# pouryashirazian/FemBrain

Hardware: AMD Instinct MI355X
Metric: FEM steps/sec (assemble+PCG) at 1M tets (higher is better)
Workload: dtype f64 arithmetic / f32 stored matrix

## Files before the change

### fembrain_amd/csrc/pcg_pipe.hip.h

```cpp
#pragma once
#include "fem_kernels.h"
#include "pcg_pipe_stream.hip.h"
#include "pcg_pipe_onchip.hip.h"
#include "pcg_pipe_mirror.h"
#include "pcg_pipe_regs.hip.h"

namespace fb {

constexpr int kPipeMaxWaves = 12;
constexpr int kPipeMaxBlocks = 256;
constexpr int kPipeSyncDoubles = 2 * 16 + 2 * kPipeMaxBlocks + 8;
constexpr int kPipeMaxProducers = 64;
constexpr int pipe_slot_bytes(bool c16) { return c16 ? 9 * 256 + 128 : 10 * 256; }
constexpr int pipe_lds_slots(bool c16) { return c16 ? 65 : 62; }
static_assert(sizeof(double) * kPipeSyncDoubles + (size_t)pipe_lds_slots(false) * pipe_slot_bytes(false) <= 160 * 1024, "LDS budget of k_pcg_pipe");
static_assert(sizeof(double) * kPipeSyncDoubles + (size_t)pipe_lds_slots(true) * pipe_slot_bytes(true) <= 160 * 1024, "LDS budget of k_pcg_pipe<c16>");
static_assert(mir_slot_bytes(true) == pipe_slot_bytes(true) && mir_slot_bytes(false) == pipe_slot_bytes(false) && mir_lds_slots(true) == pipe_lds_slots(true) &&
              mir_lds_slots(false) == pipe_lds_slots(false) && kMirWaves == kPipeMaxWaves, "the LDS window's planner sees the kernel's LDS");
static_assert(pipe_lds_slots(true) * pipe_slot_bytes(true) / 4 < 65536 && pipe_lds_slots(false) * pipe_slot_bytes(false) / 4 < 65536, "16-bit LDS word addresses of the mirror layers");

struct PipeArgs {
  unsigned long long* post;
  unsigned int* flags;
  unsigned int* error;
// ... 177 lines not shown
    if (lane == 0) { mw[w].d = d; mw[w].m = m; mw[w].width = width; }
  }
  __syncthreads();
  if (threadIdx.x == 0) ok = count > 0 && mir_wg_layout(mw, count, klt, c16, 0, false) ? 1 : 0;
  __syncthreads();
  for (int pass = 0; pass < 2; pass++) {
    if (ok && w < count) {
      int e = 0;
      for (int k = 0; k < mw[w].m; k++) e += __popcll(__ballot(mir_lane_addr(slice_off, colidx, first, mw, w, k, lane, lo, hi, c16) < 0));
      if (lane == 0) cnt[w] = e;
    }
    __syncthreads();
    if (threadIdx.x == 0 && ok) {
      int E = 0;
      for (int v = 0; v < count; v++) E += cnt[v];
      if (pass == 0) ok = E <= kMirPoolMax && mir_wg_layout(mw, count, klt, c16, E, true) ? 1 : 0;
      else ok = mir_wg_gains(mw, count, klt, c16) ? 1 : 0;
    }
    __syncthreads();
  }
  if (threadIdx.x == 0) {
    if (!ok) mir_wg_plain(mw, count, klt, c16);
    int E = 0, layers = 0, fewest = 1 << 30, held = 0;
    for (int v = 0; v < count; v++) {
      const int e = ok ? cnt[v] : 0;
      cnt[v] = E;
      E += e; layers += mw[v].m; fewest = min(fewest, mw[v].p); held += mir_reg_slots(mw[v], regs);
    }
    if (held > 0) atomicAdd(&stats[3], held);
    wg_out[b] = make_int2(mir_pool_at(mw, count, c16) / 4, E);
    atomicAdd(&stats[0], layers); atomicAdd(&stats[1], E);
    if (count > 0) atomicMin(&stats[2], fewest);
  }
  __syncthreads();
  if (w < count) {
    const int sl = first + w, pool_at = mir_pool_at(mw, count, c16) / 4;
    int e = cnt[w];
    for (int k = 0; k < mw[w].m; k++) {
      int addr = mir_lane_addr(slice_off, colidx, first, mw, w, k, lane, lo, hi, c16);
      const unsigned long long miss = __ballot(addr < 0);
      if (addr < 0) {
        const int idx = e + __popcll(miss & ((1ULL << lane) - 1ULL));
        pool_src[(size_t)b * kMirPoolMax + idx] = (slice_off[sl] + mw[w].a + k) * 9 * 64 + lane;
        addr = pool_at + (idx >> 6) * 9 * 64 + (idx & 63);
      }
      e += __popcll(miss);
      addr_out[((size_t)sl * kMirMax + k) * 64 + lane] = (unsigned short)addr;
    }
  }
  if (w < kMirWaves && lane == 0)
    wave_out[(size_t)b * kMirWaves + w] = w < count ? make_int4(mw[w].a | mw[w].m << 8 | mw[w].p << 16, mw[w].at, mw[w].tab, mir_reg_slots(mw[w], regs)) : make_int4(0, 0, 0, 0);
}

template <bool SERVE_PRIO = false>
__device__ __forceinline__ void pipe_collect_posts(const PipeArgs& pa, unsigned int sums, int nb, int lane, int stride, int l0, long long t0, long long t_limit, bool& failed,
                                                   double& t0s, double& t1s) {
  const unsigned long long* post = pa.post + (size_t)(sums & 1u) * nb * 4;
  for (int b = l0; b - lane < nb && !failed; b += stride) {
    const bool mine = b < nb;
    uint4 q4[2] = {make_uint4(0, 0, 0, 0), make_uint4(0, 0, 0, 0)};
    for (;;) {
      bool ok = true;
      if (mine) {
        asm volatile("global_load_dwordx4 %0, %2, off sc1\n\tglobal_load_dwordx4 %1, %2, off offset:16 sc1\n\ts_waitcnt vmcnt(0)"
                     : "=&v"(q4[0]), "=&v"(q4[1]) : "v"(post + (size_t)b * 4) : "memory");
        ok = q4[0].y == sums && q4[0].w == sums && q4[1].y == sums && q4[1].w == sums;
      }
      if (__ballot(!ok) == 0ULL) break;
      if constexpr (SERVE_PRIO) pipe_setprio<0>();
      if (ld_sc1_u32(pa.error) != 0u || wall_clock64() - t0 > t_limit) { failed = true; break; }
      __builtin_amdgcn_s_sleep(1);
    }
    if constexpr (SERVE_PRIO) pipe_setprio<1>();
    if (mine && !failed) {
      t0s += __longlong_as_double((long long)(((unsigned long long)q4[0].x << 32) | (unsigned long long)q4[0].z));
      t1s += __longlong_as_double((long long)(((unsigned long long)q4[1].x << 32) | (unsigned long long)q4[1].z));
    }
  }
}

__global__ __launch_bounds__(256) void k_gather_lines(int n_slices, int step, const int* __restrict__ slice_off, const int* __restrict__ colidx,
                                                      unsigned long long* __restrict__ out) {
  const int lane = threadIdx.x & 63;
  const int wave = (int)((blockIdx.x * blockDim.x + threadIdx.x) >> 6), n_waves = (int)((gridDim.x * blockDim.x) >> 6);
  unsigned long long planes = 0, records = 0, slots = 0;
  for (int s = wave * step; s < n_slices; s += n_waves * step) {
    for (int slot = slice_off[s]; slot < slice_off[s + 1]; slot++) {
      const unsigned int col = (unsigned int)colidx[(size_t)slot * 64 + lane];
      const unsigned int kp = col >> 4, k0 = (col * 24u) >> 7, k1 = (col * 24u + 23u) >> 7;
      bool first_p = true, first_0 = true, first_1 = k1 != k0;
      for (int l = 0; l < 64; l++) {
        const unsigned int op = __builtin_amdgcn_readlane(kp, l), o0 = __builtin_amdgcn_readlane(k0, l), o1 = __builtin_amdgcn_readlane(k1, l);
        if (l < lane) {
          first_p = first_p && op != kp;
          first_0 = first_0 && o0 != k0 && o1 != k0;
          first_1 = first_1 && o0 != k1 && o1 != k1;
        }
      }
      planes += __popcll(__ballot(first_p));
      records += __popcll(__ballot(first_0)) + __popcll(__ballot(first_1));
      slots++;
    }
  }
  if (lane == 0 && slots) { atomicAdd(out, planes); atomicAdd(out + 1, records); atomicAdd(out + 2, slots); }
}

}
#include "pcg_shard_box.hip.h"
namespace fb {

}
#define FB_PIPE_KERNEL k_pcg_pipe
#define FB_PIPE_KERNEL_ATTR
#define FB_PIPE_KERNEL_HOLDS false
#include "pcg_pipe_kernel.h"
#undef FB_PIPE_KERNEL
#undef FB_PIPE_KERNEL_ATTR
#undef FB_PIPE_KERNEL_HOLDS
#define FB_PIPE_KERNEL k_pcg_pipe_regs
#define FB_PIPE_KERNEL_ATTR __attribute__((amdgpu_num_vgpr(FB_PIPE_REGS_VGPR_PAIRS)))
#define FB_PIPE_KERNEL_HOLDS true
#include "pcg_pipe_kernel.h"
#undef FB_PIPE_KERNEL
// ... 3 lines not shown
```

### fembrain_amd/csrc/pcg_pipe2.hip.h

```cpp
#pragma once
#include "pcg_pipe.hip.h"

namespace fb {

constexpr int kPipe2LdsWordsPerRow = 24;
constexpr int kPipe2SliceBytes = kPipe2LdsWordsPerRow * 64 * 4;
constexpr int kPipe2Klt = 4;
__host__ __device__ constexpr int pipe2_lds_slots(int count, bool c16) {
  return (160 * 1024 - (int)sizeof(double) * kPipeSyncDoubles - (count + 1) * kPipe2SliceBytes) / pipe_slot_bytes(c16) > 0
             ? (160 * 1024 - (int)sizeof(double) * kPipeSyncDoubles - (count + 1) * kPipe2SliceBytes) / pipe_slot_bytes(c16) : 0;
}

template <bool C16, bool SHARD, bool XYZ = false>
__global__ __launch_bounds__(64 * kPipeMaxWaves) void k_pcg_pipe2(SellView sv, const float* __restrict__ vals, const float* __restrict__ dlo,
                                                                  const double* __restrict__ invdiag, const double* __restrict__ bvec,
                                                                  double* __restrict__ xg, double* __restrict__ rg, double* __restrict__ wg,
                                                                  double* __restrict__ zg, double* __restrict__ sg, double* __restrict__ pg,
                                                                  CGState* __restrict__ st, PipeArgs pa, ShardArgs sa) {
  static_assert(!SHARD || !C16, "a shard's columns are 32-bit local ids");
  static_assert(!SHARD || !XYZ, "a shard publishes planes");
  extern __shared__ double lds[];
  double* wsum = lds;
  double* gath = lds + 32;
  double* bc = gath + 2 * kPipeMaxBlocks;
// ... 41 lines not shown
#pragma unroll
      for (int j = 0; j < 9; j++) lv[(k * kValWords + j) * 64] = __float_as_uint(vk[j * 64]);
      if constexpr (C16) lc[k * 64] = sv.coldelta[((size_t)so[h] + k) * 64 + lane];
      else lv[(k * 10 + 9) * 64] = (unsigned int)sv.colidx[((size_t)so[h] + k) * 64 + lane];
    }
  }
  double iv[2][3] = {{0, 0, 0}, {0, 0, 0}};
#pragma unroll
  for (int h = 0; h < 2; h++) {
    float m6[6] = {0, 0, 0, 0, 0, 0};
    if (rvalid[h]) {
      const float* l = dlo + (size_t)(row[h] >> 6) * 9 * 64 + lane;
      m6[0] = l[0 * 64]; m6[1] = l[1 * 64]; m6[2] = l[2 * 64]; m6[3] = l[4 * 64]; m6[4] = l[5 * 64]; m6[5] = l[8 * 64];
#pragma unroll
      for (int a = 0; a < 3; a++) iv[h][a] = invdiag[3 * (size_t)row[h] + a];
    }
#pragma unroll
    for (int k = 0; k < 6; k++) *lds_f(h, k) = m6[k];
#pragma unroll
    for (int k = 0; k < 9; k++) *lds_d(h, k) = 0.0;
  }
  const int n_prod = pa.prod_count[blockIdx.x];
  int my_prod = -1;
  if (wv == 0 && n_prod >= 0 && lane < n_prod) my_prod = pa.producers[(size_t)blockIdx.x * kPipeMaxProducers + lane];

  unsigned int send_mask = 0u;
  ShardBoxLayout BL = {};
  if constexpr (SHARD) { send_mask = sa.wg_send_mask[blockIdx.x]; BL = shard_box_layout(sa.halo_cap); }
  unsigned int pub = pa.seqs[0], sums = pa.seqs[1];
  const long long t_limit = pa.timeout_ticks;
  bool failed = false;

  const size_t xs = XYZ ? 1 : pa.n_pad, cs = XYZ ? 3 : 1;
  auto publish = [&](const double vin[2][3]) {
    pub++;
    double* pl = pa.planes + (size_t)(pub & 1u) * 3 * pa.n_pad;
#pragma unroll
    for (int h = 0; h < 2; h++)
      if (rvalid[h]) {
        if constexpr (XYZ) {
          st_sc1_xyz(pl + 3 * (size_t)row[h], vin[h][0], vin[h][1], vin[h][2]);
        } else {
#pragma unroll
          for (int a = 0; a < 3; a++) st_sc1_f64(pl + a * xs + cs * (size_t)row[h], vin[h][a]);
        }
        if constexpr (SHARD) shard_send_row(sa, BL, pub, send_beg[h], send_end[h], vin[h]);
      }
  };
  auto product = [&](const double vin[2][3], double y[2][3], bool post_sums, bool late_acquire) {
    double* pl = pa.planes + (size_t)(pub & 1u) * 3 * pa.n_pad;
    asm volatile("s_waitcnt vmcnt(0)" ::: "memory");
    __syncthreads();
    if (post_sums) sums++;
    if (wv != 0 && live[0] && pa.prefetch_slots > 0 && width[0] > KL[0]) {
      int so_k = so[0] + KL[0];
      asm volatile("" : "+s"(so_k));
      pipe_prefetch_values(min(pa.prefetch_slots, width[0] - KL[0]), ((unsigned int)so_k * 9u * 64u + (unsigned int)lane) * (unsigned int)sizeof(float), vals);
    }
    if constexpr (SHARD) {
      if (spare) shard_service_product(sa, BL, pa, pub, pl, nb, lane, send_mask, t_limit, bc, failed);
    }
    if (wv == 0) {
      if (lane == 0) st_sc1_u32(pa.flags + blockIdx.x, pub);
      if (post_sums && lane < 2) {
        double t = 0.0;
        for (int w = 0; w < n_waves; w++) t += wsum[lane * 16 + w];
        const unsigned long long bits = (unsigned long long)__double_as_longlong(t), tag = (unsigned long long)sums << 32;
        unsigned long long* post = pa.post + ((size_t)(sums & 1u) * nb + blockIdx.x) * 4 + 2 * lane;
        st_sc1_u64(post, (bits >> 32) | tag);
        st_sc1_u64(post + 1, (bits & 0xffffffffULL) | tag);
      }
      if (!late_acquire) __builtin_amdgcn_fence(__ATOMIC_ACQUIRE, "agent");
      const long long t0 = wall_clock64();
      if (n_prod >= 0) {
        for (;;) {
          bool ok = true;
          if (my_prod >= 0) ok = (int)(ld_sc1_u32(pa.flags + my_prod) - pub) >= 0;
          if (__ballot(!ok) == 0ULL) break;
          if (ld_sc1_u32(pa.error) != 0u || wall_clock64() - t0 > t_limit) { failed = true; break; }
          __builtin_amdgcn_s_sleep(1);
        }
      } else if constexpr (SHARD) {
        shard_poll_all(sa, pa, pub, nb, lane, t0, t_limit, failed);
      } else {
        for (int b = 4 * lane; b - 4 * lane < nb && !failed; b += 256) {
          for (;;) {
            bool ok = true;
            if (b < nb) {
              const uint4 f = ld_sc1_u128(pa.flags + b);
              ok = (int)(f.x - pub) >= 0 && (b + 1 >= nb || (int)(f.y - pub) >= 0) && (b + 2 >= nb || (int)(f.z - pub) >= 0) && (b + 3 >= nb || (int)(f.w - pub) >= 0);
            }
            if (__ballot(!ok) == 0ULL) break;
            if (ld_sc1_u32(pa.error) != 0u || wall_clock64() - t0 > t_limit) { failed = true; break; }
            __builtin_amdgcn_s_sleep(1);
          }
        }
      }
      if (failed && lane == 0) st_sc1_u32(pa.error, 1u);
      if (late_acquire) __builtin_amdgcn_fence(__ATOMIC_ACQUIRE, "agent");
      asm volatile("s_waitcnt vmcnt(0)" ::: "memory");
      if (lane == 0) bc[3] = (failed || ld_sc1_u32(pa.error) != 0u) ? 1.0 : 0.0;
    }
    __syncthreads();
    if (uniform_flag(bc[3] != 0.0 || (SHARD && bc[4] != 0.0))) { failed = true; return; }
#pragma unroll
    for (int h = 0; h < 2; h++) {
      double y0 = 0, y1 = 0, y2 = 0;
      if (rvalid[h]) {
        const double l00 = (double)*lds_f(h, 0), l01 = (double)*lds_f(h, 1), l02 = (double)*lds_f(h, 2), l11 = (double)*lds_f(h, 3), l12 = (double)*lds_f(h, 4),
                     l22 = (double)*lds_f(h, 5);
        y0 = l00 * vin[h][0] + l01 * vin[h][1] + l02 * vin[h][2];
        y1 = l01 * vin[h][0] + l11 * vin[h][1] + l12 * vin[h][2];
        y2 = l02 * vin[h][0] + l12 * vin[h][1] + l22 * vin[h][2];
      }
      if (live[h]) {
        const unsigned int* lv = (const unsigned int*)lres[h] + lane;
        const short* lc = (const short*)(lres[h] + (size_t)klt[h] * 9 * 256) + lane;
#pragma unroll
        for (int k = 0; k < kPipe2Klt; k++) if (k < KL[h]) {
          const unsigned int* lk = lv + (size_t)k * kValWords * 64;
          unsigned int col;
          if constexpr (C16) col = (unsigned int)(row[h] + (int)lc[k * 64]); else col = lk[9 * 64];
          const double* xp = pl + cs * (size_t)col;
          const double x0 = xp[0], x1 = xp[xs], x2 = xp[2 * xs];
          y0 += (double)__uint_as_float(lk[0 * 64]) * x0 + (double)__uint_as_float(lk[1 * 64]) * x1 + (double)__uint_as_float(lk[2 * 64]) * x2;
          y1 += (double)__uint_as_float(lk[3 * 64]) * x0 + (double)__uint_as_float(lk[4 * 64]) * x1 + (double)__uint_as_float(lk[5 * 64]) * x2;
          y2 += (double)__uint_as_float(lk[6 * 64]) * x0 + (double)__uint_as_float(lk[7 * 64]) * x1 + (double)__uint_as_float(lk[8 * 64]) * x2;
        }
      }
      if (live[h] && width[h] > KL[h]) {
        int so_k = so[h] + KL[h];
        asm volatile("" : "+s"(so_k));
        pipe_stream_slots<C16, XYZ>(width[h] - KL[h], ((unsigned int)so_k * 9u * 64u + (unsigned int)lane) * (unsigned int)sizeof(float),
                               ((unsigned int)so_k * 64u + (unsigned int)lane) * (unsigned int)(C16 ? sizeof(short) : sizeof(int)), vals,
                               C16 ? (const void*)sv.coldelta : (const void*)sv.colidx, pl, pl + xs, pl + 2 * xs, row[h], y0, y1, y2);
      }
      y[h][0] = y0; y[h][1] = y1; y[h][2] = y2;
    }
  };

  double rr[2][3] = {{0, 0, 0}, {0, 0, 0}}, wr[2][3] = {{0, 0, 0}, {0, 0, 0}}, sr[2][3] = {{0, 0, 0}, {0, 0, 0}};
  double rho0 = 0.0, eps2 = pa.eps2, gamma_old = 1.0, alpha_old = 1.0;
  int iter = 0, max_iter = pa.max_iter;
  enum { PH_WARM_X = 0, PH_INIT_W = 1, PH_ITER = 2, PH_REFRESH_X = 3, PH_REFRESH_W = 4 };
  int phase = PH_ITER;
  bool fresh = pa.start != 0;
  if (pa.start == 0) {
#pragma unroll
    for (int h = 0; h < 2; h++)
      if (rvalid[h]) {
        const size_t dof = 3 * (size_t)row[h];
#pragma unroll
        for (int a = 0; a < 3; a++) {
          rr[h][a] = rg[dof + a]; wr[h][a] = wg[dof + a]; sr[h][a] = sg[dof + a];
// ... 27 lines not shown
  while (!failed) {
    if (phase == PH_ITER && it_done >= pa.n_iters) break;
    double vin[2][3];
#pragma unroll
    for (int h = 0; h < 2; h++)
#pragma unroll
      for (int a = 0; a < 3; a++)
        vin[h][a] = (phase == PH_WARM_X || phase == PH_REFRESH_X) ? *lds_d(h, a) : (phase == PH_ITER ? iv[h][a] * wr[h][a] : iv[h][a] * rr[h][a]);
    if (!published) publish(vin);
    published = false;
    if (phase == PH_ITER) {
      double a0 = 0.0, a1 = 0.0;
#pragma unroll
      for (int h = 0; h < 2; h++) {
        const double u[3] = {iv[h][0] * rr[h][0], iv[h][1] * rr[h][1], iv[h][2] * rr[h][2]};
        a0 += rr[h][0] * u[0] + rr[h][1] * u[1] + rr[h][2] * u[2];
        a1 += wr[h][0] * u[0] + wr[h][1] * u[1] + wr[h][2] * u[2];
      }
      a0 = wave_sum(a0); a1 = wave_sum(a1);
      int wvo = wv;
      asm volatile("" : "+v"(wvo));
      if (lane == 0) { wsum[wvo] = a0; wsum[16 + wvo] = a1; }
    }
    double y[2][3];
    product(vin, y, phase == PH_ITER, phase != PH_ITER || unsettled);
    unsettled = phase != PH_ITER;
    if (failed) break;
    if (phase == PH_WARM_X || phase == PH_REFRESH_X) {
#pragma unroll
      for (int h = 0; h < 2; h++) {
        unsigned int d3 = 3u * (unsigned int)(rvalid[h] ? row[h] : 0);
        asm volatile("" : "+v"(d3));
#pragma unroll
        for (int a = 0; a < 3; a++) rr[h][a] = rvalid[h] ? bvec[d3 + a] - y[h][a] : 0.0;
      }
      phase = phase == PH_WARM_X ? PH_INIT_W : PH_REFRESH_W;
      continue;
    }
    if (phase != PH_ITER) {
#pragma unroll
      for (int h = 0; h < 2; h++)
#pragma unroll
        for (int a = 0; a < 3; a++) wr[h][a] = y[h][a];
      phase = PH_ITER;
      continue;
    }
    if constexpr (SHARD) {
      if (spare) shard_rank_sums(sa, BL, pa, sums, nb, lane, t_limit, bc, failed);
      __syncthreads();
    } else if (pa.service) {
      if (wv == n_waves - 1) {
        const long long t0 = wall_clock64();
        double t0s = 0, t1s = 0;
        pipe_collect_posts(pa, sums, nb, lane, 64, lane, t0, t_limit, failed, t0s, t1s);
        failed = uniform_flag(failed);
        if (failed && lane == 0) st_sc1_u32(pa.error, 1u);
        t0s = wave_sum(t0s); t1s = wave_sum(t1s);
        if (lane == 0) { bc[0] = t0s; bc[1] = t1s; bc[2] = (failed || ld_sc1_u32(pa.error) != 0u) ? 1.0 : 0.0; }
      }
      __syncthreads();
    } else {
      const int pollers = min(n_waves, 4);
      if (wv < pollers) {
        const long long t0 = wall_clock64();
        const unsigned long long* post = pa.post + (size_t)(sums & 1u) * nb * 4;
        for (int b = wv * 64 + lane; b - lane < nb && !failed; b += pollers * 64) {
          const bool mine = b < nb;
          uint4 q4[2] = {make_uint4(0, 0, 0, 0), make_uint4(0, 0, 0, 0)};
          for (;;) {
            bool ok = true;
            if (mine) {
              asm volatile("global_load_dwordx4 %0, %2, off sc1\n\tglobal_load_dwordx4 %1, %2, off offset:16 sc1\n\ts_waitcnt vmcnt(0)"
                           : "=&v"(q4[0]), "=&v"(q4[1]) : "v"(post + (size_t)b * 4) : "memory");
              ok = q4[0].y == sums && q4[0].w == sums && q4[1].y == sums && q4[1].w == sums;
            }
            if (__ballot(!ok) == 0ULL) break;
            if (ld_sc1_u32(pa.error) != 0u || wall_clock64() - t0 > t_limit) { failed = true; break; }
            __builtin_amdgcn_s_sleep(1);
          }
          if (mine && !failed) {
            gath[b] = __longlong_as_double((long long)(((unsigned long long)q4[0].x << 32) | (unsigned long long)q4[0].z));
            gath[kPipeMaxBlocks + b] = __longlong_as_double((long long)(((unsigned long long)q4[1].x << 32) | (unsigned long long)q4[1].z));
          }
        }
        if (failed && lane == 0) { st_sc1_u32(pa.error, 1u); bc[4] = 1.0; }
      }
      __syncthreads();
      if (wv == 0) {
        double t0s = 0, t1s = 0;
        int l0 = lane;
        asm volatile("" : "+v"(l0));
        for (int b = l0; b < nb; b += 64) { t0s += gath[b]; t1s += gath[kPipeMaxBlocks + b]; }
        t0s = wave_sum(t0s); t1s = wave_sum(t1s);
        if (lane == 0) { bc[0] = t0s; bc[1] = t1s; bc[2] = (bc[4] != 0.0 || ld_sc1_u32(pa.error) != 0u) ? 1.0 : 0.0; }
      }
      __syncthreads();
    }
    if (uniform_flag(bc[2] != 0.0)) { failed = true; break; }
    gamma = uniform_f64(bc[0]);
    const double delta = uniform_f64(bc[1]);
    if (fresh) rho0 = gamma;
    if (!(gamma > eps2 * rho0) || iter >= max_iter) { done = true; break; }
    double alpha, beta;
    if (fresh) { beta = 0.0; alpha = gamma / delta; }
    else { beta = gamma / gamma_old; alpha = gamma / (delta - beta * gamma / alpha_old); }
    fresh = false;
    iter++;
    it_done++;
    gamma_old = gamma; alpha_old = alpha;
    const bool refresh = iter % 30 == 0;
    double zn[2][3];
#pragma unroll
    for (int h = 0; h < 2; h++)
#pragma unroll
      for (int a = 0; a < 3; a++) {
        zn[h][a] = y[h][a] + beta * *lds_d(h, 6 + a);
        *lds_d(h, 6 + a) = zn[h][a];
        sr[h][a] = wr[h][a] + beta * sr[h][a];
      }
    if (!refresh) {
      double m[2][3];
#pragma unroll
      for (int h = 0; h < 2; h++)
#pragma unroll
        for (int a = 0; a < 3; a++) { wr[h][a] = wr[h][a] - alpha * zn[h][a]; m[h][a] = iv[h][a] * wr[h][a]; }
      publish(m);
      published = true;
    }
#pragma unroll
    for (int h = 0; h < 2; h++)
#pragma unroll
      for (int a = 0; a < 3; a++) {
        const double pn = iv[h][a] * rr[h][a] + beta * *lds_d(h, 3 + a);
        *lds_d(h, 3 + a) = pn;
        *lds_d(h, a) = *lds_d(h, a) + alpha * pn;
      }
    if (refresh) {
      phase = PH_REFRESH_X;
    } else {
#pragma unroll
      for (int h = 0; h < 2; h++)
#pragma unroll
        for (int a = 0; a < 3; a++) rr[h][a] = rr[h][a] - alpha * sr[h][a];
    }
  }
  if (failed) return;
  const bool capped = done && gamma > eps2 * rho0;
// ... 32 lines not shown
```

### fembrain_amd/csrc/pcg_pipe_kernel.h

```cpp
namespace fb {

template <typename MT, bool C16, int WMAX, int KLT, bool TIMING, bool SHARD, bool BJ = false, bool HELP = false, bool XYZ = false, bool AHEAD = false, int REGS = 0,
          int PRIO = 0>
__global__ __launch_bounds__(64 * WMAX) FB_PIPE_KERNEL_ATTR void FB_PIPE_KERNEL(SellView sv, const MT* __restrict__ vals, const MT* __restrict__ dlo,
                                                        const double* __restrict__ invdiag, const double* __restrict__ bvec, double* __restrict__ xg,
                                                        double* __restrict__ rg, double* __restrict__ wg, double* __restrict__ zg,
                                                        double* __restrict__ sg, double* __restrict__ pg, CGState* __restrict__ st, PipeArgs pa,
                                                        ShardArgs sa) {
  static_assert(!SHARD || (!C16 && !TIMING), "a shard's columns are 32-bit local ids; the phase clocks are built for the unsharded kernel");
  static_assert(!BJ || (!SHARD && !TIMING), "block-Jacobi is for unsharded handles");
  static_assert(!HELP || (!SHARD && !BJ), "helper wavefronts: unsharded handles, the Jacobi preconditioner");
  static_assert(!AHEAD || (!SHARD && !HELP), "run-ahead: unsharded handles without helper wavefronts (add_helpers needs the barrier)");
  static_assert((REGS > 0) == FB_PIPE_KERNEL_HOLDS, "register slots: k_pcg_pipe_regs, and only there");
  static_assert(REGS == 0 || (AHEAD && !TIMING && !BJ && !XYZ && WMAX == 12 && (KLT == 6 || KLT == 7) && REGS <= kPipeRegsMax),
                "register slots: the run-ahead LDS-window instantiations");
  static_assert(PRIO >= 0 && PRIO <= 3 && (PRIO == 0 || (AHEAD && !BJ && !XYZ && WMAX == 12 && (REGS > 0 || (TIMING && KLT == 6)))),
                "wavefront priority: the register-slot kernels and the TIMING (12, 6) run-ahead kernel");
  constexpr bool kProgress = PRIO == 1 || PRIO == 3;
  static_assert(sizeof(MT) == 4, "k_pcg_pipe keeps part of the matrix in LDS as fp32 words and streams the rest as fp32");
  extern __shared__ double lds[];
  double* wsum = lds;
  double* gath = lds + 32;
  double* bc = gath + 2 * kPipeMaxBlocks;
  unsigned int* const tot_seq = (unsigned int*)(bc + 6);
// ... 118 lines not shown
    const bool helper = !live && !spare && tk.x >= 0;
    own_k1 = __builtin_amdgcn_readfirstlane(live ? tk.z : width);
    help_mask = (unsigned int)__builtin_amdgcn_readfirstlane(live ? tk.w : 0);
    help_sl = __builtin_amdgcn_readfirstlane(helper ? first + tk.x : -1);
    hk0 = __builtin_amdgcn_readfirstlane(helper ? tk.y : 0); hk1 = __builtin_amdgcn_readfirstlane(helper ? tk.z : 0);
    help_idx = __builtin_amdgcn_readfirstlane(helper ? tk.w : 0);
    help_so = __builtin_amdgcn_readfirstlane(sv.slice_off[help_sl < 0 ? 0 : help_sl]);
  }
  const int n_prod = pa.prod_count[blockIdx.x];
  int my_prod = -1;
  if (wv == 0 && n_prod >= 0 && lane < n_prod) my_prod = pa.producers[(size_t)blockIdx.x * kPipeMaxProducers + lane];

  unsigned int send_mask = 0u;
  ShardBoxLayout BL = {};
  if constexpr (SHARD) { send_mask = sa.wg_send_mask[blockIdx.x]; BL = shard_box_layout(sa.halo_cap); }
  unsigned int pub = pa.seqs[0], sums = pa.seqs[1];
  const long long t_limit = pa.timeout_ticks;
  bool failed = false;
  long long tm[TIMING ? 7 : 1] = {0}, tprev = TIMING ? wall_clock64() : 0;
  auto seam = [&](int k, long long& t) { if (TIMING) { const long long u = wall_clock64(); tm[k] += u - t; t = u; } };
  auto lap = [&](int k) { if (TIMING) { const long long t = wall_clock64(); tm[k] += t - tprev; tprev = t; } };

  const bool plain_cand = !SHARD && pa.plain_local != 0 && pa.prod_xcd[blockIdx.x] == 0;
  bool through = true, xcc_known = false;
  unsigned int my_xcc = 0u;
  if constexpr (!SHARD) {
    asm volatile("s_getreg_b32 %0, hwreg(HW_REG_XCC_ID, 0, 4)" : "=s"(my_xcc));
    if (threadIdx.x == 0) st_sc1_u32(pa.xcc + blockIdx.x, ((pub + 1u) << 4) | my_xcc);
  }
  static_assert(!XYZ || HELP, "the node-by-node vector comes with the table-driven instantiation");
  const size_t xs = XYZ ? 1 : pa.n_pad, cs = XYZ ? 3 : 1;
  auto publish = [&](const double* vin) {
    pub++;
    double* pl = pa.planes + (size_t)(pub & 1u) * 3 * pa.n_pad;
    if (rvalid) {
      if (XYZ && through) {
        st_sc1_xyz(pl + 3 * (size_t)row, vin[0], vin[1], vin[2]);
      } else if (through) {
#pragma unroll
        for (int a = 0; a < 3; a++) st_sc1_f64(pl + a * xs + cs * (size_t)row, vin[a]);
      } else {
#pragma unroll
        for (int a = 0; a < 3; a++) pl[a * xs + cs * (size_t)row] = vin[a];
      }
      if constexpr (SHARD) shard_send_row(sa, BL, pub, send_beg, send_end, vin);
    }
  };
  auto product = [&](const double* vin, double* y, bool post_sums, bool late_acquire) {
    double* pl = pa.planes + (size_t)(pub & 1u) * 3 * pa.n_pad;
    asm volatile("s_waitcnt vmcnt(0)" ::: "memory");
    __syncthreads();
    lap(0);
    if (post_sums) sums++;
    if (REGS == 0 && wv != 0 && live && pa.prefetch_slots > 0 && (mir_a > 0 || own_k1 > k_after)) {
      int so_k = so + (mir_a > 0 ? 0 : k_after);
      asm volatile("" : "+s"(so_k));
      pipe_prefetch_values(min(pa.prefetch_slots, mir_a > 0 ? mir_a : own_k1 - k_after), ((unsigned int)so_k * 9u * 64u + (unsigned int)lane) * (unsigned int)sizeof(float), vals);
    }
    if constexpr (REGS > 0) {
      if (wv != 0 && live && pa.prefetch_slots > 0 && (n_front > 0 || own_k1 > k_behind)) {
        int so_k = so + (n_front > 0 ? 0 : k_behind);
        asm volatile("" : "+s"(so_k));
        pipe_prefetch_values_low(min(pa.prefetch_slots, n_front > 0 ? n_front : own_k1 - k_behind), ((unsigned int)so_k * 9u * 64u + (unsigned int)lane) * (unsigned int)sizeof(float), vals);
      }
    }
    if constexpr (SHARD) {
      if (spare) shard_service_product(sa, BL, pa, pub, pl, nb, lane, send_mask, t_limit, bc, failed);
    }
    if (wv == 0) {
      if (lane == 0) st_sc1_u32(pa.flags + blockIdx.x, pub);
      if (post_sums && lane < 2) {
        double t = 0.0;
        for (int w = 0; w < n_waves; w++) t += wsum[lane * 16 + w];
        const unsigned long long bits = (unsigned long long)__double_as_longlong(t), tag = (unsigned long long)sums << 32;
        unsigned long long* post = pa.post + ((size_t)(sums & 1u) * nb + blockIdx.x) * 4 + 2 * lane;
        st_sc1_u64(post, (bits >> 32) | tag);
        st_sc1_u64(post + 1, (bits & 0xffffffffULL) | tag);
      }
      if (!late_acquire) __builtin_amdgcn_fence(__ATOMIC_ACQUIRE, "agent");
      const long long t0 = wall_clock64();
      if (n_prod >= 0) {
        for (;;) {
          bool ok = true;
          if (my_prod >= 0) ok = (int)(ld_sc1_u32(pa.flags + my_prod) - pub) >= 0;
          if (__ballot(!ok) == 0ULL) break;
          if (ld_sc1_u32(pa.error) != 0u || wall_clock64() - t0 > t_limit) { failed = true; break; }
          __builtin_amdgcn_s_sleep(1);
        }
      } else if constexpr (SHARD) {
        shard_poll_all(sa, pa, pub, nb, lane, t0, t_limit, failed);
      } else {
        for (int b = 4 * lane; b - 4 * lane < nb && !failed; b += 256) {
          for (;;) {
            bool ok = true;
            if (b < nb) {
              const uint4 f = ld_sc1_u128(pa.flags + b);
              ok = (int)(f.x - pub) >= 0 && (b + 1 >= nb || (int)(f.y - pub) >= 0) && (b + 2 >= nb || (int)(f.z - pub) >= 0) && (b + 3 >= nb || (int)(f.w - pub) >= 0);
            }
            if (__ballot(!ok) == 0ULL) break;
            if (ld_sc1_u32(pa.error) != 0u || wall_clock64() - t0 > t_limit) { failed = true; break; }
            __builtin_amdgcn_s_sleep(1);
          }
        }
      }
      if (failed && lane == 0) st_sc1_u32(pa.error, 1u);
      if (late_acquire) __builtin_amdgcn_fence(__ATOMIC_ACQUIRE, "agent");
      if (plain_cand && !xcc_known && !failed) {
        const bool same = my_prod < 0 || ld_sc1_u32(pa.xcc + my_prod) == ((pub << 4) | my_xcc);
        const bool all_same = __ballot(!same) == 0ULL;
        if (lane == 0) bc[5] = all_same ? 1.0 : 0.0;
      }
      asm volatile("s_waitcnt vmcnt(0)" ::: "memory");
      if (lane == 0) bc[3] = (failed || ld_sc1_u32(pa.error) != 0u) ? 1.0 : 0.0;
    }
    __syncthreads();
    lap(1);
    if (uniform_flag(bc[3] != 0.0 || (SHARD && bc[4] != 0.0))) { failed = true; return; }
    if (plain_cand && !xcc_known) { through = !uniform_flag(bc[5] != 0.0); xcc_known = true; }
    if constexpr (kProgress) { if (uniform_flag(live)) pipe_setprio<3>(); }
    if constexpr (PRIO == 2) { if (uniform_flag(live && wv >= 8)) pipe_setprio<1>(); }
    double y0 = 0, y1 = 0, y2 = 0;
    if (rvalid) {
      MT u00 = m00, u01 = m01, u02 = m02, u11 = m11, u12 = m12, u22 = m22;
      asm volatile("" : "+v"(u00), "+v"(u01), "+v"(u02), "+v"(u11), "+v"(u12), "+v"(u22));
      const double l00 = (double)u00, l01 = (double)u01, l02 = (double)u02, l11 = (double)u11, l12 = (double)u12, l22 = (double)u22;
      y0 = l00 * vin[0] + l01 * vin[1] + l02 * vin[2];
      y1 = l01 * vin[0] + l11 * vin[1] + l12 * vin[2];
      y2 = l02 * vin[0] + l12 * vin[1] + l22 * vin[2];
    }
    long long tseam = tprev;
    if (live) {
      if constexpr (kMir) {
        if (REGS == 0 && mir_a > 0) {
          int so_k = so;
          asm volatile("" : "+s"(so_k));
          pipe_stream_slots<C16, XYZ>(mir_a, ((unsigned int)so_k * 9u * 64u + (unsigned int)lane) * (unsigned int)sizeof(float),
                                      ((unsigned int)so_k * 64u + (unsigned int)lane) * (unsigned int)(C16 ? sizeof(short) : sizeof(int)), vals,
                                      C16 ? (const void*)sv.coldelta : (const void*)sv.colidx, pl, pl + xs, pl + 2 * xs, row, y0, y1, y2);
        }
        if constexpr (REGS > 0) {
          if (n_front > 0) {
            int so_k = so;
            asm volatile("" : "+s"(so_k));
            pipe_stream_slots_low<C16>(n_front, ((unsigned int)so_k * 9u * 64u + (unsigned int)lane) * (unsigned int)sizeof(float),
                                       ((unsigned int)so_k * 64u + (unsigned int)lane) * (unsigned int)(C16 ? sizeof(short) : sizeof(int)), vals,
                                       C16 ? (const void*)sv.coldelta : (const void*)sv.colidx, pl, pl + xs, pl + 2 * xs, row, y0, y1, y2);
          }
        }
        if constexpr (kProgress) pipe_setprio<2>();
        seam(5, tseam);
        const char* lbase = (const char*)(lds + kPipeSyncDoubles);
        if constexpr (REGS > 0) {
          pipe_onchip_slots_regs<C16, kProgress>(reg_f, mir_m, max(KL, 0), reg_b, (const unsigned int*)(lbase + mir_tab) + lane, (const unsigned short*)(lbase + mir_tab) + lane, lres, lcd,
                                      lbase, pl, pl + xs, pl + 2 * xs, row, y0, y1, y2);
        } else
        pipe_onchip_slots<C16, kProgress>(mir_m, max(KL, 0), (const unsigned int*)(lbase + mir_tab) + lane, (const unsigned short*)(lbase + mir_tab) + lane, lres, lcd, lbase, pl, pl + xs,
                               pl + 2 * xs, row, y0, y1, y2);
        if constexpr (kProgress) pipe_setprio<0>();
      }
      if (sizeof(MT) == 4 && KLT >= 16) {
        double gx[KLT][3];
#pragma unroll
        for (int k = 0; k < KLT; k++) {
          const unsigned int col = k < KL ? lds_col(k) : 0u;
          const double* xp = pl + cs * (size_t)col;
          gx[k][0] = k < KL ? xp[0] : 0.0; gx[k][1] = k < KL ? xp[xs] : 0.0; gx[k][2] = k < KL ? xp[2 * xs] : 0.0;
// ... 127 lines not shown
  while (!failed) {
    if (phase == PH_ITER && it_done >= pa.n_iters) break;
    double vin[3];
    if (phase == PH_WARM_X || phase == PH_REFRESH_X) {
#pragma unroll
      for (int a = 0; a < 3; a++) vin[a] = xr[a];
    } else if (phase == PH_ITER) {
      precond(wr, vin);
    } else {
      precond(rr, vin);
    }
    if (!published) publish(vin);
    published = false;
    if (phase == PH_ITER) {
      double u[3];
      precond(rr, u);
      double a0 = rr[0] * u[0] + rr[1] * u[1] + rr[2] * u[2];
      double a1 = wr[0] * u[0] + wr[1] * u[1] + wr[2] * u[2];
      a0 = wave_sum(a0); a1 = wave_sum(a1);
      int wvo = wv;
      asm volatile("" : "+v"(wvo));
      if (lane == 0) { wsum[wvo] = a0; wsum[16 + wvo] = a1; }
    }
    double y[3];
    product(vin, y, phase == PH_ITER, phase != PH_ITER || unsettled);
    unsettled = phase != PH_ITER;
    if (failed) break;
    if constexpr (HELP) if (phase != PH_ITER) {
      __syncthreads();
      add_helpers(y);
    }
    if (phase == PH_WARM_X || phase == PH_REFRESH_X) {
      unsigned int d3 = 3u * (unsigned int)(rvalid ? row : 0);
      asm volatile("" : "+v"(d3));
#pragma unroll
      for (int a = 0; a < 3; a++) rr[a] = rvalid ? bvec[d3 + a] - y[a] : 0.0;
      phase = phase == PH_WARM_X ? PH_INIT_W : PH_REFRESH_W;
      continue;
    }
    if (phase != PH_ITER) {
#pragma unroll
      for (int a = 0; a < 3; a++) wr[a] = y[a];
      phase = PH_ITER;
      continue;
    }
    if constexpr (SHARD) {
      if (spare) shard_rank_sums(sa, BL, pa, sums, nb, lane, t_limit, bc, failed);
      __syncthreads();
    } else if (AHEAD || pa.service) {
      if (wv == n_waves - 1) {
        if constexpr (PRIO == 3) pipe_setprio<1>();
        const long long t0 = wall_clock64();
        double t0s = 0, t1s = 0;
        pipe_collect_posts<PRIO == 3>(pa, sums, nb, lane, 64, lane, t0, t_limit, failed, t0s, t1s);
        failed = uniform_flag(failed);
        if (failed && lane == 0) st_sc1_u32(pa.error, 1u);
        t0s = wave_sum(t0s); t1s = wave_sum(t1s);
        if (lane == 0) {
          bc[0] = t0s; bc[1] = t1s; bc[2] = (failed || ld_sc1_u32(pa.error) != 0u) ? 1.0 : 0.0;
          if constexpr (AHEAD) __hip_atomic_store(tot_seq, sums, __ATOMIC_RELEASE, __HIP_MEMORY_SCOPE_WORKGROUP);
        }
        if constexpr (PRIO == 3) pipe_setprio<0>();
      }
      if constexpr (AHEAD) {
        while ((unsigned int)__builtin_amdgcn_readfirstlane((int)__hip_atomic_load(tot_seq, __ATOMIC_ACQUIRE, __HIP_MEMORY_SCOPE_WORKGROUP)) != sums) __builtin_amdgcn_s_sleep(1);
      } else {
        __syncthreads();
      }
    } else {
      const int pollers = min(n_waves, 4);
      if (wv < pollers) {
        const long long t0 = wall_clock64();
        const unsigned long long* post = pa.post + (size_t)(sums & 1u) * nb * 4;
        for (int b = wv * 64 + lane; b - lane < nb && !failed; b += pollers * 64) {
          const bool mine = b < nb;
          uint4 q4[2] = {make_uint4(0, 0, 0, 0), make_uint4(0, 0, 0, 0)};
          for (;;) {
            bool ok = true;
            if (mine) {
              asm volatile("global_load_dwordx4 %0, %2, off sc1\n\tglobal_load_dwordx4 %1, %2, off offset:16 sc1\n\ts_waitcnt vmcnt(0)"
                           : "=&v"(q4[0]), "=&v"(q4[1]) : "v"(post + (size_t)b * 4) : "memory");
              ok = q4[0].y == sums && q4[0].w == sums && q4[1].y == sums && q4[1].w == sums;
            }
            if (__ballot(!ok) == 0ULL) break;
            if (ld_sc1_u32(pa.error) != 0u || wall_clock64() - t0 > t_limit) { failed = true; break; }
            __builtin_amdgcn_s_sleep(1);
          }
          if (mine && !failed) {
            gath[b] = __longlong_as_double((long long)(((unsigned long long)q4[0].x << 32) | (unsigned long long)q4[0].z));
            gath[kPipeMaxBlocks + b] = __longlong_as_double((long long)(((unsigned long long)q4[1].x << 32) | (unsigned long long)q4[1].z));
          }
        }
        if (failed && lane == 0) { st_sc1_u32(pa.error, 1u); bc[4] = 1.0; }
      }
      __syncthreads();
      if (wv == 0) {
        double t0s = 0, t1s = 0;
        int l0 = lane;
        asm volatile("" : "+v"(l0));
        for (int b = l0; b < nb; b += 64) { t0s += gath[b]; t1s += gath[kPipeMaxBlocks + b]; }
        t0s = wave_sum(t0s); t1s = wave_sum(t1s);
        if (lane == 0) { bc[0] = t0s; bc[1] = t1s; bc[2] = (bc[4] != 0.0 || ld_sc1_u32(pa.error) != 0u) ? 1.0 : 0.0; }
      }
      __syncthreads();
    }
    lap(3);
    if (uniform_flag(bc[2] != 0.0)) { failed = true; break; }
    if constexpr (HELP) add_helpers(y);
    gamma = uniform_f64(bc[0]);
    const double delta = uniform_f64(bc[1]);
    if (fresh) rho0 = gamma;
    if (!(gamma > eps2 * rho0) || iter >= max_iter) { done = true; break; }
    double alpha, beta;
    if (fresh) { beta = 0.0; alpha = gamma / delta; }
    else { beta = gamma / gamma_old; alpha = gamma / (delta - beta * gamma / alpha_old); }
    fresh = false;
    iter++;
    it_done++;
    gamma_old = gamma; alpha_old = alpha;
    const bool refresh = iter % 30 == 0;
#pragma unroll
    for (int a = 0; a < 3; a++) {
      zr[a] = y[a] + beta * zr[a];
      sr[a] = wr[a] + beta * sr[a];
    }
    if (!refresh) {
      double m[3];
#pragma unroll
      for (int a = 0; a < 3; a++) wr[a] = wr[a] - alpha * zr[a];
      precond(wr, m);
      publish(m);
      published = true;
    }
    if constexpr (BJ) {
      double ur[3];
      precond(rr, ur);
#pragma unroll
      for (int a = 0; a < 3; a++) pr[a] = ur[a] + beta * pr[a];
    } else {
#pragma unroll
      for (int a = 0; a < 3; a++) pr[a] = iv[a] * rr[a] + beta * pr[a];
    }
#pragma unroll
    for (int a = 0; a < 3; a++) xr[a] = xr[a] + alpha * pr[a];
    if (refresh) {
      phase = PH_REFRESH_X;
    } else {
#pragma unroll
      for (int a = 0; a < 3; a++) rr[a] = rr[a] - alpha * sr[a];
    }
    lap(4);
  }
  if (TIMING && lane == 0) {
    unsigned long long* tw = (unsigned long long*)pa.timing + ((size_t)blockIdx.x * kPipeMaxWaves + wv) * kPipeTimingSlots;
    for (int k = 0; k < 5; k++) atomicAdd(tw + k, (unsigned long long)tm[k]);
// ... 33 lines not shown
```

Measured before the change: 76.74.

## Shorten persistent PCG barrier critical path: offload sums store, overlap error polling

Moves the per-block dot-product post (store_sums) from wave 0 to another wave (service or wave 1), so wave 0 only publishes its flag before polling. Error-flag loads are issued alongside the flag/post polling loads rather than serially after them, and that value is reused instead of reloading. For non-shard paths the agent acquire fence becomes a bare buffer_inv sc1. This shortens the serialized latency of each grid-wide sync but relies on weaker ordering assumptions, and there is no longer a guaranteed order between a block's sums post and its flag store.

```diff
diff --git a/fembrain_amd/csrc/pcg_pipe.hip.h b/fembrain_amd/csrc/pcg_pipe.hip.h
--- a/fembrain_amd/csrc/pcg_pipe.hip.h
+++ b/fembrain_amd/csrc/pcg_pipe.hip.h
@@ -253,23 +253,26 @@
     wave_out[(size_t)b * kMirWaves + w] = w < count ? make_int4(mw[w].a | mw[w].m << 8 | mw[w].p << 16, mw[w].at, mw[w].tab, mir_reg_slots(mw[w], regs)) : make_int4(0, 0, 0, 0);
 }
 
-template <bool SERVE_PRIO = false>
+template <bool SERVE_PRIO = false, bool ERR_ALONG = false>
 __device__ __forceinline__ void pipe_collect_posts(const PipeArgs& pa, unsigned int sums, int nb, int lane, int stride, int l0, long long t0, long long t_limit, bool& failed,
-                                                   double& t0s, double& t1s) {
+                                                   double& t0s, double& t1s, unsigned int* err = nullptr) {
   const unsigned long long* post = pa.post + (size_t)(sums & 1u) * nb * 4;
   for (int b = l0; b - lane < nb && !failed; b += stride) {
     const bool mine = b < nb;
     uint4 q4[2] = {make_uint4(0, 0, 0, 0), make_uint4(0, 0, 0, 0)};
     for (;;) {
       bool ok = true;
+      unsigned int e_now = 0u;
+      if constexpr (ERR_ALONG) e_now = ld_sc1_u32(pa.error);
       if (mine) {
         asm volatile("global_load_dwordx4 %0, %2, off sc1\n\tglobal_load_dwordx4 %1, %2, off offset:16 sc1\n\ts_waitcnt vmcnt(0)"
                      : "=&v"(q4[0]), "=&v"(q4[1]) : "v"(post + (size_t)b * 4) : "memory");
         ok = q4[0].y == sums && q4[0].w == sums && q4[1].y == sums && q4[1].w == sums;
       }
+      if constexpr (ERR_ALONG) *err = e_now = (unsigned int)__builtin_amdgcn_readfirstlane((int)e_now);
       if (__ballot(!ok) == 0ULL) break;
       if constexpr (SERVE_PRIO) pipe_setprio<0>();
-      if (ld_sc1_u32(pa.error) != 0u || wall_clock64() - t0 > t_limit) { failed = true; break; }
+      if ((ERR_ALONG ? e_now : ld_sc1_u32(pa.error)) != 0u || wall_clock64() - t0 > t_limit) { failed = true; break; }
       __builtin_amdgcn_s_sleep(1);
     }
     if constexpr (SERVE_PRIO) pipe_setprio<1>();
diff --git a/fembrain_amd/csrc/pcg_pipe2.hip.h b/fembrain_amd/csrc/pcg_pipe2.hip.h
--- a/fembrain_amd/csrc/pcg_pipe2.hip.h
+++ b/fembrain_amd/csrc/pcg_pipe2.hip.h
@@ -117,16 +117,7 @@
     asm volatile("s_waitcnt vmcnt(0)" ::: "memory");
     __syncthreads();
     if (post_sums) sums++;
-    if (wv != 0 && live[0] && pa.prefetch_slots > 0 && width[0] > KL[0]) {
-      int so_k = so[0] + KL[0];
-      asm volatile("" : "+s"(so_k));
-      pipe_prefetch_values(min(pa.prefetch_slots, width[0] - KL[0]), ((unsigned int)so_k * 9u * 64u + (unsigned int)lane) * (unsigned int)sizeof(float), vals);
-    }
-    if constexpr (SHARD) {
-      if (spare) shard_service_product(sa, BL, pa, pub, pl, nb, lane, send_mask, t_limit, bc, failed);
-    }
-    if (wv == 0) {
-      if (lane == 0) st_sc1_u32(pa.flags + blockIdx.x, pub);
+    auto store_sums = [&]() {
       if (post_sums && lane < 2) {
         double t = 0.0;
         for (int w = 0; w < n_waves; w++) t += wsum[lane * 16 + w];
@@ -135,28 +126,62 @@
         st_sc1_u64(post, (bits >> 32) | tag);
         st_sc1_u64(post + 1, (bits & 0xffffffffULL) | tag);
       }
-      if (!late_acquire) __builtin_amdgcn_fence(__ATOMIC_ACQUIRE, "agent");
+    };
+    const int storer = (SHARD || n_waves == 1) ? 0 : (pa.service ? n_waves - 1 : 1);
+    if constexpr (!SHARD) {
+      if (wv == storer && storer != 0) store_sums();
+    }
+    if (wv != 0 && live[0] && pa.prefetch_slots > 0 && width[0] > KL[0]) {
+      int so_k = so[0] + KL[0];
+      asm volatile("" : "+s"(so_k));
+      pipe_prefetch_values(min(pa.prefetch_slots, width[0] - KL[0]), ((unsigned int)so_k * 9u * 64u + (unsigned int)lane) * (unsigned int)sizeof(float), vals);
+    }
+    if constexpr (SHARD) {
+      if (spare) shard_service_product(sa, BL, pa, pub, pl, nb, lane, send_mask, t_limit, bc, failed);
+    }
+    if (wv == 0) {
+      if (lane == 0) st_sc1_u32(pa.flags + blockIdx.x, pub);
+      if (SHARD || storer == 0) store_sums();
+      if (!late_acquire) {
+        if constexpr (SHARD) __builtin_amdgcn_fence(__ATOMIC_ACQUIRE, "agent");
+        else asm volatile("buffer_inv sc1" ::: "memory");
+      }
       const long long t0 = wall_clock64();
-      if (n_prod >= 0) {
+      unsigned int err = 0u;
+      if constexpr (SHARD) {
+        if (n_prod >= 0) {
+          for (;;) {
+            bool ok = true;
+            if (my_prod >= 0) ok = (int)(ld_sc1_u32(pa.flags + my_prod) - pub) >= 0;
+            if (__ballot(!ok) == 0ULL) break;
+            if (ld_sc1_u32(pa.error) != 0u || wall_clock64() - t0 > t_limit) { failed = true; break; }
+            __builtin_amdgcn_s_sleep(1);
+          }
+        } else {
+          shard_poll_all(sa, pa, pub, nb, lane, t0, t_limit, failed);
+        }
+      } else if (n_prod >= 0) {
         for (;;) {
           bool ok = true;
+          const unsigned int e = ld_sc1_u32(pa.error);
           if (my_prod >= 0) ok = (int)(ld_sc1_u32(pa.flags + my_prod) - pub) >= 0;
+          err = e;
           if (__ballot(!ok) == 0ULL) break;
-          if (ld_sc1_u32(pa.error) != 0u || wall_clock64() - t0 > t_limit) { failed = true; break; }
+          if (err != 0u || wall_clock64() - t0 > t_limit) { failed = true; break; }
           __builtin_amdgcn_s_sleep(1);
         }
-      } else if constexpr (SHARD) {
-        shard_poll_all(sa, pa, pub, nb, lane, t0, t_limit, failed);
       } else {
         for (int b = 4 * lane; b - 4 * lane < nb && !failed; b += 256) {
           for (;;) {
             bool ok = true;
+            err = ld_sc1_u32(pa.error);
             if (b < nb) {
               const uint4 f = ld_sc1_u128(pa.flags + b);
               ok = (int)(f.x - pub) >= 0 && (b + 1 >= nb || (int)(f.y - pub) >= 0) && (b + 2 >= nb || (int)(f.z - pub) >= 0) && (b + 3 >= nb || (int)(f.w - pub) >= 0);
             }
+            err = (unsigned int)__builtin_amdgcn_readfirstlane((int)err);
             if (__ballot(!ok) == 0ULL) break;
-            if (ld_sc1_u32(pa.error) != 0u || wall_clock64() - t0 > t_limit) { failed = true; break; }
+            if (err != 0u || wall_clock64() - t0 > t_limit) { failed = true; break; }
             __builtin_amdgcn_s_sleep(1);
           }
         }
@@ -164,7 +189,7 @@
       if (failed && lane == 0) st_sc1_u32(pa.error, 1u);
       if (late_acquire) __builtin_amdgcn_fence(__ATOMIC_ACQUIRE, "agent");
       asm volatile("s_waitcnt vmcnt(0)" ::: "memory");
-      if (lane == 0) bc[3] = (failed || ld_sc1_u32(pa.error) != 0u) ? 1.0 : 0.0;
+      if (lane == 0) bc[3] = (failed || (SHARD ? ld_sc1_u32(pa.error) : err) != 0u) ? 1.0 : 0.0;
     }
     __syncthreads();
     if (uniform_flag(bc[3] != 0.0 || (SHARD && bc[4] != 0.0))) { failed = true; return; }
@@ -298,15 +323,17 @@
       if (wv == n_waves - 1) {
         const long long t0 = wall_clock64();
         double t0s = 0, t1s = 0;
-        pipe_collect_posts(pa, sums, nb, lane, 64, lane, t0, t_limit, failed, t0s, t1s);
+        unsigned int err = 0u;
+        pipe_collect_posts<false, true>(pa, sums, nb, lane, 64, lane, t0, t_limit, failed, t0s, t1s, &err);
         failed = uniform_flag(failed);
         if (failed && lane == 0) st_sc1_u32(pa.error, 1u);
         t0s = wave_sum(t0s); t1s = wave_sum(t1s);
-        if (lane == 0) { bc[0] = t0s; bc[1] = t1s; bc[2] = (failed || ld_sc1_u32(pa.error) != 0u) ? 1.0 : 0.0; }
+        if (lane == 0) { bc[0] = t0s; bc[1] = t1s; bc[2] = (failed || err != 0u) ? 1.0 : 0.0; }
       }
       __syncthreads();
     } else {
       const int pollers = min(n_waves, 4);
+      unsigned int err = 0u;
       if (wv < pollers) {
         const long long t0 = wall_clock64();
         const unsigned long long* post = pa.post + (size_t)(sums & 1u) * nb * 4;
@@ -315,13 +342,15 @@
           uint4 q4[2] = {make_uint4(0, 0, 0, 0), make_uint4(0, 0, 0, 0)};
           for (;;) {
             bool ok = true;
+            err = ld_sc1_u32(pa.error);
             if (mine) {
               asm volatile("global_load_dwordx4 %0, %2, off sc1\n\tglobal_load_dwordx4 %1, %2, off offset:16 sc1\n\ts_waitcnt vmcnt(0)"
                            : "=&v"(q4[0]), "=&v"(q4[1]) : "v"(post + (size_t)b * 4) : "memory");
               ok = q4[0].y == sums && q4[0].w == sums && q4[1].y == sums && q4[1].w == sums;
             }
+            err = (unsigned int)__builtin_amdgcn_readfirstlane((int)err);
             if (__ballot(!ok) == 0ULL) break;
-            if (ld_sc1_u32(pa.error) != 0u || wall_clock64() - t0 > t_limit) { failed = true; break; }
+            if (err != 0u || wall_clock64() - t0 > t_limit) { failed = true; break; }
             __builtin_amdgcn_s_sleep(1);
           }
           if (mine && !failed) {
@@ -338,7 +367,7 @@
         asm volatile("" : "+v"(l0));
         for (int b = l0; b < nb; b += 64) { t0s += gath[b]; t1s += gath[kPipeMaxBlocks + b]; }
         t0s = wave_sum(t0s); t1s = wave_sum(t1s);
-        if (lane == 0) { bc[0] = t0s; bc[1] = t1s; bc[2] = (bc[4] != 0.0 || ld_sc1_u32(pa.error) != 0u) ? 1.0 : 0.0; }
+        if (lane == 0) { bc[0] = t0s; bc[1] = t1s; bc[2] = (bc[4] != 0.0 || err != 0u) ? 1.0 : 0.0; }
       }
       __syncthreads();
     }
diff --git a/fembrain_amd/csrc/pcg_pipe_kernel.h b/fembrain_amd/csrc/pcg_pipe_kernel.h
--- a/fembrain_amd/csrc/pcg_pipe_kernel.h
+++ b/fembrain_amd/csrc/pcg_pipe_kernel.h
@@ -194,23 +194,7 @@
     __syncthreads();
     lap(0);
     if (post_sums) sums++;
-    if (REGS == 0 && wv != 0 && live && pa.prefetch_slots > 0 && (mir_a > 0 || own_k1 > k_after)) {
-      int so_k = so + (mir_a > 0 ? 0 : k_after);
-      asm volatile("" : "+s"(so_k));
-      pipe_prefetch_values(min(pa.prefetch_slots, mir_a > 0 ? mir_a : own_k1 - k_after), ((unsigned int)so_k * 9u * 64u + (unsigned int)lane) * (unsigned int)sizeof(float), vals);
-    }
-    if constexpr (REGS > 0) {
-      if (wv != 0 && live && pa.prefetch_slots > 0 && (n_front > 0 || own_k1 > k_behind)) {
-        int so_k = so + (n_front > 0 ? 0 : k_behind);
-        asm volatile("" : "+s"(so_k));
-        pipe_prefetch_values_low(min(pa.prefetch_slots, n_front > 0 ? n_front : own_k1 - k_behind), ((unsigned int)so_k * 9u * 64u + (unsigned int)lane) * (unsigned int)sizeof(float), vals);
-      }
-    }
-    if constexpr (SHARD) {
-      if (spare) shard_service_product(sa, BL, pa, pub, pl, nb, lane, send_mask, t_limit, bc, failed);
-    }
-    if (wv == 0) {
-      if (lane == 0) st_sc1_u32(pa.flags + blockIdx.x, pub);
+    auto store_sums = [&]() {
       if (post_sums && lane < 2) {
         double t = 0.0;
         for (int w = 0; w < n_waves; w++) t += wsum[lane * 16 + w];
@@ -219,28 +203,69 @@
         st_sc1_u64(post, (bits >> 32) | tag);
         st_sc1_u64(post + 1, (bits & 0xffffffffULL) | tag);
       }
-      if (!late_acquire) __builtin_amdgcn_fence(__ATOMIC_ACQUIRE, "agent");
+    };
+    const int storer = SHARD ? 0 : (AHEAD ? n_waves - 1 : (n_waves == 1 ? 0 : (pa.service ? n_waves - 1 : 1)));
+    if constexpr (!SHARD) {
+      if (wv == storer && storer != 0) store_sums();
+    }
+    if (REGS == 0 && wv != 0 && live && pa.prefetch_slots > 0 && (mir_a > 0 || own_k1 > k_after)) {
+      int so_k = so + (mir_a > 0 ? 0 : k_after);
+      asm volatile("" : "+s"(so_k));
+      pipe_prefetch_values(min(pa.prefetch_slots, mir_a > 0 ? mir_a : own_k1 - k_after), ((unsigned int)so_k * 9u * 64u + (unsigned int)lane) * (unsigned int)sizeof(float), vals);
+    }
+    if constexpr (REGS > 0) {
+      if (wv != 0 && live && pa.prefetch_slots > 0 && (n_front > 0 || own_k1 > k_behind)) {
+        int so_k = so + (n_front > 0 ? 0 : k_behind);
+        asm volatile("" : "+s"(so_k));
+        pipe_prefetch_values_low(min(pa.prefetch_slots, n_front > 0 ? n_front : own_k1 - k_behind), ((unsigned int)so_k * 9u * 64u + (unsigned int)lane) * (unsigned int)sizeof(float), vals);
+      }
+    }
+    if constexpr (SHARD) {
+      if (spare) shard_service_product(sa, BL, pa, pub, pl, nb, lane, send_mask, t_limit, bc, failed);
+    }
+    if (wv == 0) {
+      if (lane == 0) st_sc1_u32(pa.flags + blockIdx.x, pub);
+      if (SHARD || (!AHEAD && storer == 0)) store_sums();
+      if (!late_acquire) {
+        if constexpr (SHARD) __builtin_amdgcn_fence(__ATOMIC_ACQUIRE, "agent");
+        else asm volatile("buffer_inv sc1" ::: "memory");
+      }
       const long long t0 = wall_clock64();
-      if (n_prod >= 0) {
+      unsigned int err = 0u;
+      if constexpr (SHARD) {
+        if (n_prod >= 0) {
+          for (;;) {
+            bool ok = true;
+            if (my_prod >= 0) ok = (int)(ld_sc1_u32(pa.flags + my_prod) - pub) >= 0;
+            if (__ballot(!ok) == 0ULL) break;
+            if (ld_sc1_u32(pa.error) != 0u || wall_clock64() - t0 > t_limit) { failed = true; break; }
+            __builtin_amdgcn_s_sleep(1);
+          }
+        } else {
+          shard_poll_all(sa, pa, pub, nb, lane, t0, t_limit, failed);
+        }
+      } else if (n_prod >= 0) {
         for (;;) {
           bool ok = true;
+          const unsigned int e = ld_sc1_u32(pa.error);
           if (my_prod >= 0) ok = (int)(ld_sc1_u32(pa.flags + my_prod) - pub) >= 0;
+          err = e;
           if (__ballot(!ok) == 0ULL) break;
-          if (ld_sc1_u32(pa.error) != 0u || wall_clock64() - t0 > t_limit) { failed = true; break; }
+          if (err != 0u || wall_clock64() - t0 > t_limit) { failed = true; break; }
           __builtin_amdgcn_s_sleep(1);
         }
-      } else if constexpr (SHARD) {
-        shard_poll_all(sa, pa, pub, nb, lane, t0, t_limit, failed);
       } else {
         for (int b = 4 * lane; b - 4 * lane < nb && !failed; b += 256) {
           for (;;) {
             bool ok = true;
+            err = ld_sc1_u32(pa.error);
             if (b < nb) {
               const uint4 f = ld_sc1_u128(pa.flags + b);
               ok = (int)(f.x - pub) >= 0 && (b + 1 >= nb || (int)(f.y - pub) >= 0) && (b + 2 >= nb || (int)(f.z - pub) >= 0) && (b + 3 >= nb || (int)(f.w - pub) >= 0);
             }
+            err = (unsigned int)__builtin_amdgcn_readfirstlane((int)err);
             if (__ballot(!ok) == 0ULL) break;
-            if (ld_sc1_u32(pa.error) != 0u || wall_clock64() - t0 > t_limit) { failed = true; break; }
+            if (err != 0u || wall_clock64() - t0 > t_limit) { failed = true; break; }
             __builtin_amdgcn_s_sleep(1);
           }
         }
@@ -253,7 +278,7 @@
         if (lane == 0) bc[5] = all_same ? 1.0 : 0.0;
       }
       asm volatile("s_waitcnt vmcnt(0)" ::: "memory");
-      if (lane == 0) bc[3] = (failed || ld_sc1_u32(pa.error) != 0u) ? 1.0 : 0.0;
+      if (lane == 0) bc[3] = (failed || (SHARD ? ld_sc1_u32(pa.error) : err) != 0u) ? 1.0 : 0.0;
     }
     __syncthreads();
     lap(1);
@@ -487,12 +512,13 @@
         if constexpr (PRIO == 3) pipe_setprio<1>();
         const long long t0 = wall_clock64();
         double t0s = 0, t1s = 0;
-        pipe_collect_posts<PRIO == 3>(pa, sums, nb, lane, 64, lane, t0, t_limit, failed, t0s, t1s);
+        unsigned int err = 0u;
+        pipe_collect_posts<PRIO == 3, true>(pa, sums, nb, lane, 64, lane, t0, t_limit, failed, t0s, t1s, &err);
         failed = uniform_flag(failed);
         if (failed && lane == 0) st_sc1_u32(pa.error, 1u);
         t0s = wave_sum(t0s); t1s = wave_sum(t1s);
         if (lane == 0) {
-          bc[0] = t0s; bc[1] = t1s; bc[2] = (failed || ld_sc1_u32(pa.error) != 0u) ? 1.0 : 0.0;
+          bc[0] = t0s; bc[1] = t1s; bc[2] = (failed || err != 0u) ? 1.0 : 0.0;
           if constexpr (AHEAD) __hip_atomic_store(tot_seq, sums, __ATOMIC_RELEASE, __HIP_MEMORY_SCOPE_WORKGROUP);
         }
         if constexpr (PRIO == 3) pipe_setprio<0>();
@@ -504,6 +530,7 @@
       }
     } else {
       const int pollers = min(n_waves, 4);
+      unsigned int err = 0u;
       if (wv < pollers) {
         const long long t0 = wall_clock64();
         const unsigned long long* post = pa.post + (size_t)(sums & 1u) * nb * 4;
@@ -512,13 +539,15 @@
           uint4 q4[2] = {make_uint4(0, 0, 0, 0), make_uint4(0, 0, 0, 0)};
           for (;;) {
             bool ok = true;
+            err = ld_sc1_u32(pa.error);
             if (mine) {
               asm volatile("global_load_dwordx4 %0, %2, off sc1\n\tglobal_load_dwordx4 %1, %2, off offset:16 sc1\n\ts_waitcnt vmcnt(0)"
                            : "=&v"(q4[0]), "=&v"(q4[1]) : "v"(post + (size_t)b * 4) : "memory");
               ok = q4[0].y == sums && q4[0].w == sums && q4[1].y == sums && q4[1].w == sums;
             }
+            err = (unsigned int)__builtin_amdgcn_readfirstlane((int)err);
             if (__ballot(!ok) == 0ULL) break;
-            if (ld_sc1_u32(pa.error) != 0u || wall_clock64() - t0 > t_limit) { failed = true; break; }
+            if (err != 0u || wall_clock64() - t0 > t_limit) { failed = true; break; }
             __builtin_amdgcn_s_sleep(1);
           }
           if (mine && !failed) {
@@ -535,7 +564,7 @@
         asm volatile("" : "+v"(l0));
         for (int b = l0; b < nb; b += 64) { t0s += gath[b]; t1s += gath[kPipeMaxBlocks + b]; }
         t0s = wave_sum(t0s); t1s = wave_sum(t1s);
-        if (lane == 0) { bc[0] = t0s; bc[1] = t1s; bc[2] = (bc[4] != 0.0 || ld_sc1_u32(pa.error) != 0u) ? 1.0 : 0.0; }
+        if (lane == 0) { bc[0] = t0s; bc[1] = t1s; bc[2] = (bc[4] != 0.0 || err != 0u) ? 1.0 : 0.0; }
       }
       __syncthreads();
     }
```

Result: slower. 72.12 (-6.0%).
